# sovrasov/3d-object-detection.pytorch

Measured on AMD Instinct MI355X. Metric: regression train crops/sec @224^2 bs256 MobileNetV2, higher is better.
Workload: dtype bf16; 1 GPU; mobilenetv2 9-class Objectron keypoint regression, train step (fwd + l1/add/CE losses + bwd + AdamW), 224x224 crops, per-GPU batch 256; global_batch=256, parallelism=dp1, roofline_sampled_steps=0, rccl_ranks=0

## Files before the change

### 3d-object-detection.pytorch_amd/csrc/elementwise.hip

```cpp
#include "common.h"

namespace {

template <typename T, bool U8>
__global__ __launch_bounds__(256) void im2col_kernel(const void* __restrict__ xin, const float* __restrict__ mean,
                                                     const float* __restrict__ istd, T* __restrict__ col, int B,
                                                     int H, int W, int Ho, int Wo) {
  extern __shared__ float tile[];
  const int WP = W + 2;
  const int hp = (Ho + 1) / 2;
  const int b = blockIdx.x / hp, oy0 = (blockIdx.x % hp) * 2;
  const int iy0 = oy0 * 2 - 1;
  const int tid = threadIdx.x;
  for (int i = tid; i < 15 * 2; i += 256) {
    const int rr = i >> 1;
    tile[rr * WP + ((i & 1) ? W + 1 : 0)] = 0.f;
  }
  if constexpr (U8) {
    const unsigned char* xu = reinterpret_cast<const unsigned char*>(xin);
    const float mu[3] = {mean[0], mean[1], mean[2]}, is[3] = {istd[0], istd[1], istd[2]};
    const int RB = W * 3;
    if ((RB & 3) == 0) {
      const int R4 = RB >> 2;
      for (int i = tid; i < 5 * R4; i += 256) {
        const int r = i / R4, e0 = (i - r * R4) * 4;
        const int iy = iy0 + r;
        const bool ok = iy >= 0 && iy < H;
        const unsigned int u = ok ? *reinterpret_cast<const unsigned int*>(xu + ((size_t)b * H + iy) * RB + e0) : 0u;
#pragma unroll
        for (int k = 0; k < 4; ++k) {
          const int e = e0 + k, ix = e / 3, ci = e - ix * 3;
          const float m = ci == 0 ? mu[0] : (ci == 1 ? mu[1] : mu[2]), sc = ci == 0 ? is[0] : (ci == 1 ? is[1] : is[2]);
          tile[(ci * 5 + r) * WP + ix + 1] = ok ? ((float)((u >> (8 * k)) & 0xffu) * (1.0f / 255.0f) - m) * sc : 0.f;
        }
      }
    } else {
      for (int i = tid; i < 5 * RB; i += 256) {
        const int r = i / RB, e = i - r * RB, ix = e / 3, ci = e - ix * 3;
        const int iy = iy0 + r;
        float v = 0.f;
        if (iy >= 0 && iy < H) v = ((float)xu[((size_t)b * H + iy) * RB + e] * (1.0f / 255.0f) - mu[ci]) * is[ci];
        tile[(ci * 5 + r) * WP + ix + 1] = v;
      }
    }
  } else {
    const float* xf = reinterpret_cast<const float*>(xin);
    if ((W & 3) == 0) {
      const int W4 = W >> 2;
      for (int i = tid; i < 15 * W4; i += 256) {
        const int rr = i / W4, x4 = i - rr * W4, ci = rr / 5, r = rr - ci * 5;
        const int iy = iy0 + r;
        float4 v = make_float4(0.f, 0.f, 0.f, 0.f);
        if (iy >= 0 && iy < H) v = *reinterpret_cast<const float4*>(xf + (((size_t)b * 3 + ci) * H + iy) * W + x4 * 4);
        float* d = tile + rr * WP + x4 * 4 + 1;
        d[0] = v.x; d[1] = v.y; d[2] = v.z; d[3] = v.w;
      }
    } else {
      for (int i = tid; i < 15 * W; i += 256) {
        const int rr = i / W, ix = i - rr * W, ci = rr / 5, r = rr - ci * 5;
        const int iy = iy0 + r;
        tile[rr * WP + ix + 1] = (iy >= 0 && iy < H) ? xf[(((size_t)b * 3 + ci) * H + iy) * W + ix] : 0.f;
      }
    }
  }
  __syncthreads();
  const int nrow = min(2, Ho - oy0);
  for (int it = tid; it < nrow * Wo * 4; it += 256) {
    const int q = it & 3, pp = it >> 2, ro = pp / Wo, ox = pp - ro * Wo;
    float v[8];
#pragma unroll
    for (int i = 0; i < 8; ++i) {
      const int idx = q * 8 + i;
      const int ci = idx / 9, r = idx - ci * 9, ky = r / 3, kx = r - ky * 3;
      v[i] = idx < 27 ? tile[(ci * 5 + ro * 2 + ky) * WP + ox * 2 + kx] : 0.f;
    }
    Vec8<T>::store(col + (((size_t)b * Ho + oy0 + ro) * Wo + ox) * 32 + q * 8, v);
  }
}

struct EwArgs {
  const void *a, *b;
  const void* res;
  void* out;
  const float *scale, *shift;
  const float* vec;
  const float* vec2;
  float* pooled;
  double* stats;
  int act;
  int M, C, HW;
  float inv_hw;
  const T3dFold* fold;
  int mode;
  int* argmax;
};

__device__ __forceinline__ void load_affine(const EwArgs& a, int c0, float sc[8], float sh[8]) {
#pragma unroll
  for (int i = 0; i < 8; ++i) {
    sc[i] = a.scale ? a.scale[c0 + i] : 1.f;
    sh[i] = a.scale ? a.shift[c0 + i] : 0.f;
  }
}

__device__ __forceinline__ void flush_stats(float* lraw, int C, int c0, bool on, const float s1[8],
                                            const float s2[8], double* stats) {
  double* lstat = reinterpret_cast<double*>(lraw);
  for (int i = threadIdx.x; i < 2 * C; i += blockDim.x) lstat[i] = 0.0;
  __syncthreads();
  if (on) {
#pragma unroll
// ... 256 lines not shown
    }
  }
  if (a.stats) {
#pragma unroll
    for (int j = 0; j < 8; ++j) {
      red[0][slot * rowl + cgl * 8 + j] = s1[j];
      red[1][slot * rowl + cgl * 8 + j] = s2[j];
    }
    __syncthreads();
    const int t = threadIdx.x, c = blockIdx.y * rowl + t;
    if (t < rowl && c < a.C) {
      double u1 = 0.0, u2 = 0.0;
      for (int q = 0; q < nslots; ++q) {
        u1 += (double)red[0][q * rowl + t];
        u2 += (double)red[1][q * rowl + t];
      }
      double* st = a.stats + (size_t)(blockIdx.x % g_nrep) * g_rstride;
      atomicAdd(st + c, u1);
      atomicAdd(st + a.C + c, u2);
    }
  }
}

inline void fill_pro(EwArgs& a, const t3d_prologue* pro) {
  if (pro) { a.scale = pro->scale; a.shift = pro->shift; a.act = pro->act; }
}
inline int ew_grid(size_t nvec) {
  size_t g = (nvec + 255) / 256;
  return (int)(g < 1 ? 1 : (g > 2048 ? 2048 : g));
}

}

static int im2col_launch(int dtype, const void* x, bool u8, const float* mean, const float* istd, void* col, int B,
                         int H, int W, void* stream) {
  if (!x || !col || B <= 0 || H <= 0 || W <= 0 || (u8 && (!mean || !istd))) return T3D_ERR_ARG;
  const int Ho = (H + 2 - 3) / 2 + 1, Wo = (W + 2 - 3) / 2 + 1;
  const int grid = B * ((Ho + 1) / 2);
  const size_t lds = (size_t)15 * (W + 2) * sizeof(float);
  if (lds > 64 * 1024) return T3D_ERR_UNSUPPORTED;
  hipStream_t st = reinterpret_cast<hipStream_t>(stream);
#define T3D_IM2COL(T, U) \
  T3D_LAUNCH((im2col_kernel<T, U>), dim3(grid), dim3(256), lds, st, x, mean, istd, (T*)col, B, H, W, Ho, Wo)
  if (dtype == T3D_F32) {
    if (u8) T3D_IM2COL(float, true); else T3D_IM2COL(float, false);
  } else if (dtype == T3D_BF16) {
    if (u8) T3D_IM2COL(bf16_t, true); else T3D_IM2COL(bf16_t, false);
  } else if (dtype == T3D_F16) {
    if (u8) T3D_IM2COL(f16_t, true); else T3D_IM2COL(f16_t, false);
  } else {
    return T3D_ERR_ARG;
  }
#undef T3D_IM2COL
  T3D_CHECK_LAUNCH();
  return T3D_OK;
}

extern "C" int t3d_stem_im2col(int dtype, const float* x, void* col, int B, int H, int W, void* stream) {
  return im2col_launch(dtype, x, false, nullptr, nullptr, col, B, H, W, stream);
}

extern "C" int t3d_stem_im2col_u8(int dtype, const unsigned char* x, const float* mean, const float* inv_std, void* col,
                                  int B, int H, int W, void* stream) {
  return im2col_launch(dtype, x, true, mean, inv_std, col, B, H, W, stream);
}

extern "C" int t3d_bn_apply(int dtype, const void* y, const t3d_prologue* pro, const void* residual, void* z,
                            int M, int C, void* stream) {
  if (!y || !z || M <= 0 || C <= 0 || (C % 8)) return T3D_ERR_ARG;
  if (pro && pro->se) return T3D_ERR_UNSUPPORTED;
  EwArgs a{};
  a.a = y; a.res = residual; a.out = z; a.M = M; a.C = C;
  fill_pro(a, pro);
  const int grid = ew_grid((size_t)M * (C / 8));
  if ((size_t)grid * 256 < (size_t)(C / 8)) return T3D_ERR_UNSUPPORTED;
  hipStream_t st = reinterpret_cast<hipStream_t>(stream);
  a.fold = t3d_take_fold(a.scale);
  const size_t lds = a.fold ? (size_t)2 * C * sizeof(float) : 0;
  if (dtype == T3D_F32) T3D_LAUNCH(bn_apply_kernel<float>, dim3(grid), dim3(256), lds, st, a);
  else if (dtype == T3D_BF16) T3D_LAUNCH(bn_apply_kernel<bf16_t>, dim3(grid), dim3(256), lds, st, a);
  else if (dtype == T3D_F16) T3D_LAUNCH(bn_apply_kernel<f16_t>, dim3(grid), dim3(256), lds, st, a);
  else return T3D_ERR_ARG;
  T3D_CHECK_LAUNCH();
  return T3D_OK;
}

extern "C" int t3d_bn_act_bwd(int dtype, const void* dz, const void* y, const t3d_prologue* pro, void* dzp,
                              double* stats, int M, int C, void* stream) {
  if (!dz || !y || !dzp || M <= 0 || C <= 0 || (C % 8)) return T3D_ERR_ARG;
  if (pro && pro->se) return T3D_ERR_UNSUPPORTED;
  EwArgs a{};
  a.a = dz; a.b = y; a.out = dzp; a.stats = stats; a.M = M; a.C = C;
  fill_pro(a, pro);
  int grid = ew_grid((size_t)M * (C / 8));
  if (grid > 1024) grid = 1024;
  if ((size_t)grid * 256 < (size_t)(C / 8)) return T3D_ERR_UNSUPPORTED;
  const size_t lds = (size_t)2 * C * sizeof(double);
  hipStream_t st = reinterpret_cast<hipStream_t>(stream);
  if (dtype == T3D_F32) T3D_LAUNCH(bn_act_bwd_kernel<float>, dim3(grid), dim3(256), lds, st, a);
// ... 90 lines not shown
```

### 3d-object-detection.pytorch_amd/csrc/plan.hip

```cpp
#include <chrono>
#include <cstdio>
#include <cstdlib>
#include <cstring>
#include <string>
#include <utility>
#include <vector>

#include "common.h"

namespace {

template <class T>
inline T word_to(uint64_t v) {
  if constexpr (std::is_pointer<T>::value) {
    return reinterpret_cast<T>(static_cast<uintptr_t>(v));
  } else if constexpr (std::is_same<T, float>::value) {
    const uint32_t b = static_cast<uint32_t>(v);
    float f;
    std::memcpy(&f, &b, 4);
    return f;
  } else if constexpr (std::is_same<T, double>::value) {
    double d;
    std::memcpy(&d, &v, 8);
    return d;
  } else {
    return static_cast<T>(static_cast<int64_t>(v));
  }
}

template <class... A, size_t... I>
inline int call_words(int (*fn)(A...), const uint64_t* w, std::index_sequence<I...>) {
  return fn(word_to<A>(w[I])...);
}

template <class... A>
constexpr int arity(int (*)(A...)) { return (int)sizeof...(A); }

template <auto Fn>
struct Thunk;
template <class... A, int (*Fn)(A...)>
struct Thunk<Fn> {
  static int run(const uint64_t* w) { return call_words(Fn, w, std::index_sequence_for<A...>{}); }
};

struct Entry { const char* name; int (*run)(const uint64_t*); int nargs; };
#define T3D_E(fn) {#fn, &Thunk<&fn>::run, arity(&fn)}
const Entry kEntries[] = {
    T3D_E(t3d_dwconv_fwd), T3D_E(t3d_bn_finalize), T3D_E(t3d_bn_eval_affine), T3D_E(t3d_bn_eval_affine_batched),
    T3D_E(t3d_pwconv_fwd), T3D_E(t3d_pwconv_dgrad), T3D_E(t3d_pack_weight), T3D_E(t3d_sum_replicas_batched),
    T3D_E(t3d_set_dw_slots), T3D_E(t3d_set_exact_pool), T3D_E(t3d_sum_slots_batched), T3D_E(t3d_dwconv_bwd),
    T3D_E(t3d_pwconv_wgrad), T3D_E(t3d_pwconv_yfree_prep), T3D_E(t3d_pwconv_dgrad_yfree), T3D_E(t3d_pwconv_wgrad_yfree),
    T3D_E(t3d_pwconv_yfree_prep2), T3D_E(t3d_pwconv_bwd_yfree), T3D_E(t3d_pwconv_bwd_yfree_w), T3D_E(t3d_pwconv_wgrad_yfree_finish),
    T3D_E(t3d_bn_bwd_finalize), T3D_E(t3d_stem_im2col), T3D_E(t3d_stem_im2col_u8), T3D_E(t3d_crop_resize_u8),
    T3D_E(t3d_pwconv_fwd_mat), T3D_E(t3d_im2col), T3D_E(t3d_im2col_nchw), T3D_E(t3d_col2im_bwd), T3D_E(t3d_pack_conv_weight),
    T3D_E(t3d_unpack_conv_grad), T3D_E(t3d_maxpool_fwd), T3D_E(t3d_maxpool_bwd), T3D_E(t3d_res_relu_fwd),
    T3D_E(t3d_res_relu_bwd), T3D_E(t3d_subsample), T3D_E(t3d_ir_block_eval), T3D_E(t3d_bn_apply), T3D_E(t3d_bn_act_bwd),
    T3D_E(t3d_gap_fwd), T3D_E(t3d_gap_bwd), T3D_E(t3d_pool_fwd), T3D_E(t3d_pool_bwd), T3D_E(t3d_head_fwd),
    T3D_E(t3d_linear_fwd), T3D_E(t3d_head_fwd_all), T3D_E(t3d_head_bwd), T3D_E(t3d_head_bwd_weights), T3D_E(t3d_se_fwd),
    T3D_E(t3d_se_bwd), T3D_E(t3d_se_fwd_fused), T3D_E(t3d_se_bwd_data), T3D_E(t3d_se_bwd_weights), T3D_E(t3d_se_after_sums),
    T3D_E(t3d_se_after_apply), T3D_E(t3d_se_after_bwd), T3D_E(t3d_set_reduction_replicas), T3D_E(t3d_set_workspace), T3D_E(t3d_set_main_workspace),
    T3D_E(t3d_fold_request), T3D_E(t3d_pack_weights_batched), T3D_E(t3d_pwconv_pack_frag), T3D_E(t3d_adamw_step), T3D_E(t3d_set_grad_watch),
    T3D_E(t3d_sgd_step), T3D_E(t3d_rmsprop_step), T3D_E(t3d_adadelta_step),
    T3D_E(t3d_zero_batched), T3D_E(t3d_copy_cols), T3D_E(t3d_bn_bias_grad), T3D_E(t3d_se_bwd_affine), T3D_E(t3d_dropout_mask),
    T3D_E(t3d_loss_fwd_bwd), T3D_E(t3d_metrics_per_sample), T3D_E(t3d_iou3d), T3D_E(t3d_box_iou3d), T3D_E(t3d_ssd_decode_nms),
    T3D_E(t3d_expdw_fwd), T3D_E(t3d_track_step), T3D_E(t3d_ssd_select_rects), T3D_E(t3d_head_select), T3D_E(t3d_track_kp_to_frame),
    T3D_E(t3d_objectron_pairs), T3D_E(t3d_objectron_hitmiss), T3D_E(t3d_draw_overlays_u8),
};
#undef T3D_E
constexpr int kNumEntries = (int)(sizeof(kEntries) / sizeof(kEntries[0]));
constexpr int kMaxArgs = 24;

enum OpKind { OP_CALL = 0, OP_FORK = 1, OP_COPY_D2H = 2, OP_EVENT_RECORD = 3 };
enum ArgKind { ARG_WORD = 0, ARG_STRUCT = 1, ARG_SLOT = 2 };

struct Op {
  int kind;
  int entry;
  int nargs;
  uint64_t w[kMaxArgs];
  uint8_t ak[kMaxArgs];
  hipEvent_t ev;
  hipStream_t sig_stream;
};

}

// ... 228 lines not shown
```

### 3d-object-detection.pytorch_amd/torchdet3d/_native.py

```python
import ctypes
import os

import torch

_HERE = os.path.dirname(os.path.abspath(__file__))
LIB_PATH = os.environ.get('T3D_LIB') or os.path.join(os.path.dirname(_HERE), 'libt3d_hip.so')

W_FRAG = 0x100
F32, BF16, F16 = 0, 1, 2
ACT = {'none': 0, 'relu': 1, 'relu6': 2, 'hswish': 3}
DW_AUTO, DW_TILE, DW_ROW3, DW_PLANE7, DW_ROWK, DW_LDS = -1, 0, 1, 2, 3, 4
PW_AUTO, PW_DEEP, PW_STREAM, PW_REG32, PW_LDS, PW_TR, PW_PAIR = -1, 0, 1, 2, 3, 4, 5
PW_OP_FWD, PW_OP_FWD_STATS, PW_OP_MAT, PW_OP_DGRAD, PW_OP_WGRAD = 0, 1, 2, 3, 4
ERR_ARG, ERR_UNSUPPORTED = -1, -3
POOL = {'avg': 0, 'max': 1, 'avg+max': 2}
_P, _I, _F, _D, _L = ctypes.c_void_p, ctypes.c_int, ctypes.c_float, ctypes.c_double, ctypes.c_longlong


class BnBwd(ctypes.Structure):
    _fields_ = [('alpha', _P), ('beta', _P), ('gamma', _P), ('per_sample', _I)]


class Prologue(ctypes.Structure):
    _fields_ = [('scale', _P), ('shift', _P), ('se', _P), ('act', _I), ('se_after_act', _I)]


class LossCfg(ctypes.Structure):
    _fields_ = [(n, _F) for n in ('c_l1', 'c_mse', 'c_smoothl1', 'smoothl1_beta', 'c_add', 'c_diag', 'c_wing',
                                  'wing_w', 'wing_eps', 'c_ce', 'lam_reg', 'lam_cls')]


class BnFold(ctypes.Structure):
    _fields_ = [('kind', _I), ('C', _I), ('nrep', _I), ('rstride', _L), ('stats', _P), ('count', _D), ('gamma', _P), ('beta', _P),
                ('rm', _P), ('rv', _P), ('nbt', _P), ('momentum', _F), ('eps', _F), ('o0', _P), ('o1', _P), ('o2', _P),
                ('o3', _P), ('o4', _P), ('mean', _P), ('invstd', _P)]


class DrawStyleC(ctypes.Structure):
    _fields_ = [('rect_th', _I), ('edge_th', _I), ('kp_radius', _I), ('font_scale', _I), ('flags', _I),
                ('colors', ctypes.c_ubyte * 3 * 8)]


DRAW_IDS = 1
_PP = ctypes.POINTER(Prologue)
_BP = ctypes.POINTER(BnBwd)
_LP = ctypes.POINTER(LossCfg)

SIGNATURES = {
    't3d_version': [],
    't3d_dwconv_fwd': [_I, _P, _PP, _P, _P, _P, _P, _I, _I, _I, _I, _I, _I, _P],
    't3d_bn_finalize': [_P, _I, _D, _P, _P, _P, _P, _P, _F, _F, _P, _P, _P, _P, _P],
    't3d_bn_eval_affine': [_I, _P, _P, _P, _P, _F, _P, _P, _P],
    't3d_bn_eval_affine_batched': [_P, _I, _F, _P],
    't3d_pwconv_fwd': [_I, _P, _PP, _P, _P, _P, _P, _I, _I, _I, _I, _P],
    't3d_pwconv_dgrad': [_I, _P, _P, _BP, _P, _P, _PP, _P, _P, _P, _P, _I, _I, _I, _I, _P],
    't3d_pack_weight': [_I, _P, _P, _I, _I, _I, _P],
    't3d_sum_replicas_batched': [_P, _I, _I, _P],
    't3d_set_dw_slots': [_I, _P],
    't3d_set_exact_pool': [_I],
    't3d_set_launch_events': [_P, _P],
    't3d_sum_slots_batched': [_P, _I, _P],
    't3d_dwconv_bwd': [_I, _P, _P, _BP, _P, _P, _PP, _P, _P, _P, _P, _I, _I, _I, _I, _I, _I, _P],
    't3d_dwconv_route': [_I] * 10,
    't3d_dwconv_force_route': [_I],
    't3d_pwconv_wgrad': [_I, _P, _P, _BP, _P, _PP, _P, _I, _I, _I, _I, _P],
    't3d_pwconv_route': [_I] * 15,
    't3d_pwconv_force_route': [_I],
    't3d_pwconv_yfree_prep': [_P, _BP, _P, _P, _I, _I, _P],
    't3d_pwconv_dgrad_yfree': [_P, _P, _P, _P, _P, _PP, _P, _P, _P, _I, _I, _I, _I, _P],
    't3d_pwconv_wgrad_yfree': [_P, _P, _BP, _P, _P, _I, _I, _I, _I, _P],
    't3d_pwconv_yfree_prep2': [_P, _BP, _P, _P, _P, _I, _I, _P],
    't3d_pwconv_bwd_yfree_scratch': [_I, _I, _I],
    't3d_pwconv_bwd_yfree': [_P, _P, _P, _P, _PP, _P, _P, _P, _P, _L, _I, _I, _I, _I, _P],
    't3d_pwconv_bwd_yfree_w': [_P, _P, _P, _BP, _P, _PP, _P, _P, _P, _P, _L, _I, _I, _I, _I, _P],
    't3d_pwconv_wgrad_yfree_finish': [_P, _BP, _P, _P, _I, _I, _I, _P],
    't3d_bn_bwd_finalize': [_P, _I, _D, _P, _P, _P, _P, _P, _P, _P, _P, _P],
    't3d_stem_im2col': [_I, _P, _P, _I, _I, _I, _P],
    't3d_stem_im2col_u8': [_I, _P, _P, _P, _P, _I, _I, _I, _P],
    't3d_crop_resize_u8': [_P, _P, _P, _I, _I, _I, _I, _I, _P],
    't3d_augment_crops_u8': [_P, _L, _P, _P, _I, _I, _I, _P],
    't3d_augment_resized_u8': [_P, _L, _P, _P, _I, _I, _I, _P],
    't3d_augment_chain_crops_u8': [_P, _L, _P, _P, _P, _L, _P, _I, _I, _I, _I, _P],
    't3d_augment_chain_resized_u8': [_P, _L, _P, _P, _P, _L, _P, _I, _I, _I, _I, _P],
    't3d_pwconv_fwd_mat': [_I, _P, _PP, _P, _P, _P, _P, _P, _I, _I, _I, _I, _P],
    't3d_ssd_decode_nms': [_I, _I, _P, _P, _P, _P, _P, _P, _P, _I, _I, _F, _F, _I, _F, _F, _P, _P, _P, _P],
    't3d_track_state_bytes': [_I],
    't3d_track_lds_bytes': [_I, _I],
    't3d_track_step': [_P, _P, _P, _P, _I, _I, _I, _I, _I, _I, _D, _D, _I, _D, _D, _D, _I, _I, _P, _P, _P, _P, _P, _P],
    't3d_ssd_select_rects': [_P, _P, _I, _I, _I, _I, _F, _F, _I, _I, _D, _D, _I, _P, _P, _P, _P, _P, _P, _P],
    't3d_head_select': [_P, _P, _I, _I, _I, _P, _P, _P],
    't3d_track_kp_to_frame': [_P, _P, _P, _P, _I, _I, _P],
    't3d_draw_overlays_u8': [_P, _I, _I, _I, _P, _P, _P, _P, _P, _P, _I, _I, ctypes.POINTER(DrawStyleC), _P],
    't3d_draw_glyphs': [_P, _I],
    't3d_objectron_pairs': [_P] * 7 + [_I, _I, _I, _D, _D, _P, _P, _P],
    't3d_objectron_hitmiss': [_P] * 8 + [_I] * 5 + [_P] * 6,
    't3d_im2col': [_I, _P, _PP, _P, _I, _I, _I, _I, _I, _I, _I, _I, _P],
    't3d_im2col_nchw': [_I, _P, _P, _I, _I, _I, _I, _I, _I, _I, _I, _P],
    't3d_col2im_bwd': [_I, _P, _P, _PP, _P, _P, _I, _I, _I, _I, _I, _I, _I, _I, _P],
    't3d_pack_conv_weight': [_I, _P, _P, _I, _I, _I, _I, _P],
    't3d_unpack_conv_grad': [_P, _P, _I, _I, _I, _I, _P],
    't3d_maxpool_fwd': [_I, _P, _PP, _P, _P, _I, _I, _I, _I, _P],
    't3d_maxpool_bwd': [_I, _P, _P, _P, _PP, _P, _P, _I, _I, _I, _I, _P],
    't3d_res_relu_fwd': [_I, _P, _PP, _P, _PP, _P, _I, _I, _P],
    't3d_res_relu_bwd': [_I, _P, _P, _P, _P, _P, _P, _P, _I, _I, _P],
    't3d_subsample': [_I, _P, _P, _I, _I, _I, _I, _I, _I, _P],
    't3d_ir_block_eval': [_P, _P, _P, _P, _I, _P, _P, _P, _I, _P, _P, _P, _I, _P, _I, _I, _I, _I, _I, _I, _P],
    't3d_bn_apply': [_I, _P, _PP, _P, _P, _I, _I, _P],
    't3d_bn_act_bwd': [_I, _P, _P, _PP, _P, _P, _I, _I, _P],
    't3d_gap_fwd': [_I, _P, _PP, _P, _I, _I, _I, _P],
    't3d_gap_bwd': [_I, _P, _P, _PP, _P, _P, _I, _I, _I, _P],
    't3d_pool_fwd': [_I, _P, _PP, _I, _P, _P, _I, _I, _I, _P],
# ... 93 lines not shown
        return _raw_stream(torch.cuda.current_device())
    return torch.cuda.current_stream().cuda_stream


class KernelTimer:

    def __init__(self, only=None, prealloc=0, kernel_exact=False):
        self.only, self.rec, self.sig, self.kernel_exact = only, [], [], kernel_exact
        self.pool = [torch.cuda.Event(enable_timing=True) for _ in range(prealloc)]
        for e in self.pool:
            e.record()

    def event(self):
        return self.pool.pop() if self.pool else torch.cuda.Event(enable_timing=True)

    def per_launch(self):
        torch.cuda.synchronize()
        return [(n, sg, e0.elapsed_time(e1), nb) for (n, nb, e0, e1), sg in zip(self.rec, self.sig)]

    def summary(self):
        torch.cuda.synchronize()
        out = {}
        for name, nbytes, e0, e1 in self.rec:
            d = out.setdefault(name, dict(launches=0, ms=0.0, bytes=0))
            d['launches'] += 1
            d['ms'] += e0.elapsed_time(e1)
            d['bytes'] += nbytes or 0
        return out


timer = None
_KERNEL_TIMED = frozenset(('t3d_dwconv_fwd', 't3d_dwconv_bwd', 't3d_expdw_fwd', 't3d_pwconv_fwd', 't3d_pwconv_fwd_mat', 't3d_pwconv_dgrad',
                           't3d_pwconv_wgrad', 't3d_pwconv_dgrad_yfree', 't3d_pwconv_wgrad_yfree', 't3d_pwconv_bwd_yfree',
                           't3d_pwconv_bwd_yfree_w'))
_ABLATE = frozenset(x for x in os.environ.get('T3D_ABLATE', '').split(',') if x)


SLOT_IMGS, SLOT_GT, SLOT_CATS, SLOT_DROPOUT, SLOT_STEP, SLOT_LR, SLOT_RB_DST, SLOT_RB_EVENT, NSLOTS = range(9)
recorder = None


def call(name, *args, nbytes=None, slots=None):
    if _ABLATE and name in _ABLATE:
        return
    fn = getattr(lib(), name)
    if recorder is not None:
        recorder.add_call(name, args, nbytes, slots)
        rc = fn(*args)
        recorder.after_call()
        if rc != 0:
            raise RuntimeError(f'{name} failed with code {rc}')
        return
    t = timer
    if t is not None and (t.only is None or name in t.only):
        e0, e1 = t.event(), t.event()
        if name in _KERNEL_TIMED and t.kernel_exact:
            lib().t3d_set_launch_events(e0.cuda_event, e1.cuda_event)
            rc = fn(*args)
            lib().t3d_set_launch_events(None, None)
        else:
            e0.record()
            rc = fn(*args)
            e1.record()
        t.rec.append((name, nbytes, e0, e1))
        t.sig.append(tuple(a for a in args[:-1] if isinstance(a, int) and not isinstance(a, bool) and 0 <= a < (1 << 31)))
    else:
        rc = fn(*args)
# ... 126 lines not shown
```

### 3d-object-detection.pytorch_amd/torchdet3d/models/engine.py

```python
import math
import os

import torch

from .. import _native as N
from .arch import Arch

BN_EPS, BN_MOM = 1e-5, 0.1
NREP = 16
FUSED_EVAL_MIN_B = int(os.environ.get('T3D_FUSED_EVAL_MIN_B', '96'))
DW_SLOTS = int(os.environ.get('T3D_DW_SLOTS', '512'))
WORKSPACE_BYTES = 64 << 20
MAIN_WORKSPACE_BYTES = 16 << 20
YFREE_MIN_ELEMS = int(os.environ.get('T3D_YFREE_MIN', 8 << 20))
YFREE_MAX_K = int(os.environ.get('T3D_YFREE_MAX_K', 112))
HOOK_MIN = 1 << 20
SE_AFTER_FUSED = None
HOOK_ON_SIDE = True


def _se_after_fused_by_shape(dt, B, HW, C, R):
    if B < 8:
        return False
    if C * R <= 4096:
# ... 556 lines not shown
        finally:
            N.call('t3d_set_reduction_replicas', 1, 0)
            self._pool_exact(False)
            self._cur_nrep = None
        cur, a = sv['last_in'], self.arch
        M = sv['B'] * cur.H * cur.W
        z = torch.empty(M, a.last_c, device=self.device, dtype=self.dtype)
        N.call('t3d_bn_apply', self.dt, N.ptr(sv['yl']), sv['prol'], None, N.ptr(z), M, a.last_c, N.stream())
        return z.float().view(sv['B'], cur.H, cur.W, a.last_c).permute(0, 3, 1, 2).contiguous()

    def _features(self, imgs, train):
        a, st, dt = self.arch, N.stream(), self.dt
        u8 = imgs.dtype == torch.uint8
        assert imgs.is_cuda and imgs.dim() == 4 and ((u8 and imgs.shape[3] == 3) or (imgs.dtype == torch.float32 and imgs.shape[1] == 3))
        imgs = imgs.contiguous()
        self.training = bool(train)
        self._pack()
        if u8:
            B, H, W, _ = imgs.shape
        else:
            B, _, H, W = imgs.shape
        if train:
            self._zero_group('fwd', [[self._statbuf.data_ptr(), self._statbuf.numel() * self._statbuf.element_size()]])
        else:
            self._zero_group('fwd')
            self._eval_affines()
        sv = dict(B=B, imgs=imgs, blocks=[])
        self.saved_blocks = sv['blocks']

        Ho, Wo = (H + 2 - 3) // 2 + 1, (W + 2 - 3) // 2 + 1
        M = B * Ho * Wo
        bn0 = self.bns[a.keys.stem_bn]
        y0 = self._buf('y:stem', (M, a.stem_c))
        col = self._buf('col', (M, 32))
        if u8:
            N.call('t3d_stem_im2col_u8', dt, N.ptr(imgs), N.ptr(self.in_mean), N.ptr(self.in_istd), N.ptr(col), B, H, W, st)
        else:
            N.call('t3d_stem_im2col', dt, N.ptr(imgs), N.ptr(col), B, H, W, st)
        N.call('t3d_pwconv_fwd', dt, N.ptr(col), None, N.ptr(self.w['stem']), None, N.ptr(y0), self._st(bn0),
               M, Ho * Wo, 32, a.stem_c, st, nbytes=M * (32 + a.stem_c) * self.esz)
        pro0 = self._bn_fwd(bn0, M, a.stem_act)
        cur = _Src(y0, pro0, B, Ho, Wo, a.stem_c, raw=y0, bn=bn0, gpro=pro0)
        sv['col'], sv['stem'] = col, cur

        taps = getattr(self, '_want_taps', None)
        for i, blk in enumerate(a.blocks):
            cur = self._block_fwd(i, blk, cur, sv)
            if taps and (i + 1) in taps:
                sv.setdefault('taps', {})[i + 1] = self._resolve(cur)

        bnl = self.bns[a.keys.last_bn]
        M = cur.B * cur.H * cur.W
        yl = self._buf('y:last', (M, a.last_c))
        self._pw_from(cur, self.w[a.keys.last_w], yl, bnl, M, cur.H * cur.W, cur.C, a.last_c)
        prol = self._bn_fwd(bnl, M, a.last_act)
        pooled = self._buf('pooled', (B, a.last_c), torch.float32)
        sv.update(last_in=cur, yl=yl, prol=prol, pooled=pooled, HWl=cur.H * cur.W, bnl=bnl)
        return sv

    def _wsel(self, w, plain=True):
        f = self._frag.get(w.data_ptr()) if (plain and self.dt in (N.BF16, N.F16)) else None
        return (self.dt | N.W_FRAG, N.ptr(f)) if f is not None else (self.dt, N.ptr(w))

    def _resolve(self, src):
        if src.zbuf is not None:
            M = src.B * src.H * src.W
            self._c('t3d_bn_apply', self.dt, N.ptr(src.t), src.pro, N.ptr(src.zres), N.ptr(src.zbuf), M, src.C, N.stream(),
                    fwd=src.bn)
            src.t, src.pro, src.zres, src.zbuf = src.zbuf, None, None, None
        return src

    def _pw_from(self, x, w, y, bn_out, M, HW, K, Nn):
        st, nb = N.stream(), M * (K + Nn) * self.esz
# ... 529 lines not shown
```

### include/t3d.h

```cpp
#ifndef T3D_H_
#define T3D_H_
#include <stdint.h>
#ifdef __cplusplus
extern "C" {
#endif

enum { T3D_F32 = 0, T3D_BF16 = 1, T3D_F16 = 2 };
enum { T3D_W_FRAG = 0x100 };
enum { T3D_ACT_NONE = 0, T3D_ACT_RELU = 1, T3D_ACT_RELU6 = 2, T3D_ACT_HSWISH = 3 };
enum { T3D_OK = 0, T3D_ERR_ARG = -1, T3D_ERR_LAUNCH = -2, T3D_ERR_UNSUPPORTED = -3 };

typedef struct {
  const float* scale;
  const float* shift;
  const float* se;
  int act;
  int se_after_act;
} t3d_prologue;

int t3d_version(void);

int t3d_dwconv_fwd(int dtype, const void* x, const t3d_prologue* pro, const float* w, void* y,
                   double* stats, float* gap_sum, int B, int H, int W, int C, int k, int stride,
                   void* stream);
// ... 41 lines not shown

int t3d_pwconv_yfree_prep(const void* wt, const t3d_bnbwd* bb, void* wcat, float* cvec, int K, int N, void* stream);
int t3d_pwconv_dgrad_yfree(const void* dz, const void* x, const void* wcat, const float* cvec, const void* x_raw,
                           const t3d_prologue* pro_in, const void* residual, void* dx, double* stats, int M, int HW,
                           int K, int N, void* stream);
int t3d_pwconv_wgrad_yfree(const void* dz, const void* x, const t3d_bnbwd* bb, const void* w, float* dw, int M, int HW,
                           int K, int N, void* stream);

int t3d_pwconv_yfree_prep2(const void* wt, const t3d_bnbwd* bb, void* wcat, float* cvec, void* wd, int K, int N, void* stream);
int t3d_pwconv_bwd_yfree_w(const void* dz, const void* x, const void* wt, const t3d_bnbwd* bb, const void* x_raw,
                           const t3d_prologue* pro_in, const void* residual, void* dx, double* stats, void* scratch,
                           long long scratch_bytes, int M, int HW, int K, int N, void* stream);
int t3d_pwconv_bwd_yfree_scratch(int M, int K, int N);
int t3d_pwconv_bwd_yfree(const void* dz, const void* x, const void* wd, const void* x_raw, const t3d_prologue* pro_in,
                         const void* residual, void* dx, double* stats, void* scratch, long long scratch_bytes, int M, int HW,
                         int K, int N, void* stream);
int t3d_pwconv_wgrad_yfree_finish(void* scratch, const t3d_bnbwd* bb, const void* w, float* dw, int M, int K, int N, void* stream);

int t3d_dwconv_bwd(int dtype, const void* dz, const void* y, const t3d_bnbwd* bb, const float* w,
                   const void* x, const t3d_prologue* pro, const void* residual, void* dx, double* stats,
                   float* dw, int B, int H, int W, int C, int k, int stride, void* stream);

enum { T3D_DW_AUTO = -1, T3D_DW_TILE = 0, T3D_DW_ROW3 = 1, T3D_DW_PLANE7 = 2, T3D_DW_ROWK = 3, T3D_DW_LDS = 4 };
int t3d_dwconv_route(int backward, int dtype, int gated_input, int pooled, int B, int H, int W, int C, int k, int stride);
int t3d_dwconv_force_route(int route);

int t3d_bn_bwd_finalize(const double* stats, int C, double count, const float* gamma, const float* mean,
                        const float* invstd, float* alpha, float* beta, float* gammac, float* dgamma,
                        float* dbeta, void* stream);

int t3d_stem_im2col(int dtype, const float* x, void* col, int B, int H, int W, void* stream);
int t3d_stem_im2col_u8(int dtype, const unsigned char* x, const float* mean, const float* inv_std, void* col, int B, int H,
                       int W, void* stream);

int t3d_ir_block_eval(const void* x, const void* w1, const float* scale1, const float* shift1, int act1, const float* wdw,
                      const float* scale2, const float* shift2, int act2, const void* w2, const float* scale3,
                      const float* shift3, int residual, void* z, int B, int H, int W, int Cin, int Ce, int Cout, void* stream);

int t3d_crop_resize_u8(const unsigned char* frame, const int* rects, unsigned char* out, int n, int H, int W, int oh, int ow,
                       void* stream);

enum { T3D_AUG_FLIP = 1, T3D_AUG_LUT = 2, T3D_AUG_ROTATE = 4, T3D_AUG_SWAP_RB = 8 };
typedef struct {
  long long offset;
  int h, w;
  int flags;
  float alpha;
  float beta255;
  int reserved;
  double m[6];
} t3d_aug_sample;
int t3d_augment_crops_u8(const unsigned char* src, long long src_bytes, const void* samples, unsigned char* out, int B, int oh,
                         int ow, void* stream);

int t3d_augment_resized_u8(const unsigned char* arena, long long arena_bytes, const void* samples, unsigned char* out, int B,
                           int oh, int ow, void* stream);

enum { T3D_CHAIN_LUT = 1, T3D_CHAIN_HSV = 2, T3D_CHAIN_BRIGHTNESS = 3, T3D_CHAIN_CONTRAST = 4, T3D_CHAIN_SATURATION = 5,
       T3D_CHAIN_HUE = 6 };
enum { T3D_CHAIN_WARP2 = 1 };
enum { T3D_STAGE_MEAN = 1, T3D_STAGE_WARP = 2, T3D_STAGE_WARP2 = 4 };
#define T3D_CHAIN_MAX_OPS 8
typedef struct {
  int n_ops;
  int flags;
  int kind[T3D_CHAIN_MAX_OPS];
// ... 227 lines not shown
```

Before: 38160 crops/s.

## Fuse stem im2col, MFMA conv and BN stats into one persistent kernel

```diff
diff --git a/3d-object-detection.pytorch_amd/csrc/elementwise.hip b/3d-object-detection.pytorch_amd/csrc/elementwise.hip
--- a/3d-object-detection.pytorch_amd/csrc/elementwise.hip
+++ b/3d-object-detection.pytorch_amd/csrc/elementwise.hip
@@ -1,82 +1,6 @@
 #include "common.h"
 
 namespace {
-
-template <typename T, bool U8>
-__global__ __launch_bounds__(256) void im2col_kernel(const void* __restrict__ xin, const float* __restrict__ mean,
-                                                     const float* __restrict__ istd, T* __restrict__ col, int B,
-                                                     int H, int W, int Ho, int Wo) {
-  extern __shared__ float tile[];
-  const int WP = W + 2;
-  const int hp = (Ho + 1) / 2;
-  const int b = blockIdx.x / hp, oy0 = (blockIdx.x % hp) * 2;
-  const int iy0 = oy0 * 2 - 1;
-  const int tid = threadIdx.x;
-  for (int i = tid; i < 15 * 2; i += 256) {
-    const int rr = i >> 1;
-    tile[rr * WP + ((i & 1) ? W + 1 : 0)] = 0.f;
-  }
-  if constexpr (U8) {
-    const unsigned char* xu = reinterpret_cast<const unsigned char*>(xin);
-    const float mu[3] = {mean[0], mean[1], mean[2]}, is[3] = {istd[0], istd[1], istd[2]};
-    const int RB = W * 3;
-    if ((RB & 3) == 0) {
-      const int R4 = RB >> 2;
-      for (int i = tid; i < 5 * R4; i += 256) {
-        const int r = i / R4, e0 = (i - r * R4) * 4;
-        const int iy = iy0 + r;
-        const bool ok = iy >= 0 && iy < H;
-        const unsigned int u = ok ? *reinterpret_cast<const unsigned int*>(xu + ((size_t)b * H + iy) * RB + e0) : 0u;
-#pragma unroll
-        for (int k = 0; k < 4; ++k) {
-          const int e = e0 + k, ix = e / 3, ci = e - ix * 3;
-          const float m = ci == 0 ? mu[0] : (ci == 1 ? mu[1] : mu[2]), sc = ci == 0 ? is[0] : (ci == 1 ? is[1] : is[2]);
-          tile[(ci * 5 + r) * WP + ix + 1] = ok ? ((float)((u >> (8 * k)) & 0xffu) * (1.0f / 255.0f) - m) * sc : 0.f;
-        }
-      }
-    } else {
-      for (int i = tid; i < 5 * RB; i += 256) {
-        const int r = i / RB, e = i - r * RB, ix = e / 3, ci = e - ix * 3;
-        const int iy = iy0 + r;
-        float v = 0.f;
-        if (iy >= 0 && iy < H) v = ((float)xu[((size_t)b * H + iy) * RB + e] * (1.0f / 255.0f) - mu[ci]) * is[ci];
-        tile[(ci * 5 + r) * WP + ix + 1] = v;
-      }
-    }
-  } else {
-    const float* xf = reinterpret_cast<const float*>(xin);
-    if ((W & 3) == 0) {
-      const int W4 = W >> 2;
-      for (int i = tid; i < 15 * W4; i += 256) {
-        const int rr = i / W4, x4 = i - rr * W4, ci = rr / 5, r = rr - ci * 5;
-        const int iy = iy0 + r;
-        float4 v = make_float4(0.f, 0.f, 0.f, 0.f);
-        if (iy >= 0 && iy < H) v = *reinterpret_cast<const float4*>(xf + (((size_t)b * 3 + ci) * H + iy) * W + x4 * 4);
-        float* d = tile + rr * WP + x4 * 4 + 1;
-        d[0] = v.x; d[1] = v.y; d[2] = v.z; d[3] = v.w;
-      }
-    } else {
-      for (int i = tid; i < 15 * W; i += 256) {
-        const int rr = i / W, ix = i - rr * W, ci = rr / 5, r = rr - ci * 5;
-        const int iy = iy0 + r;
-        tile[rr * WP + ix + 1] = (iy >= 0 && iy < H) ? xf[(((size_t)b * 3 + ci) * H + iy) * W + ix] : 0.f;
-      }
-    }
-  }
-  __syncthreads();
-  const int nrow = min(2, Ho - oy0);
-  for (int it = tid; it < nrow * Wo * 4; it += 256) {
-    const int q = it & 3, pp = it >> 2, ro = pp / Wo, ox = pp - ro * Wo;
-    float v[8];
-#pragma unroll
-    for (int i = 0; i < 8; ++i) {
-      const int idx = q * 8 + i;
-      const int ci = idx / 9, r = idx - ci * 9, ky = r / 3, kx = r - ky * 3;
-      v[i] = idx < 27 ? tile[(ci * 5 + ro * 2 + ky) * WP + ox * 2 + kx] : 0.f;
-    }
-    Vec8<T>::store(col + (((size_t)b * Ho + oy0 + ro) * Wo + ox) * 32 + q * 8, v);
-  }
-}
 
 struct EwArgs {
   const void *a, *b;
@@ -399,39 +323,6 @@
 
 }
 
-static int im2col_launch(int dtype, const void* x, bool u8, const float* mean, const float* istd, void* col, int B,
-                         int H, int W, void* stream) {
-  if (!x || !col || B <= 0 || H <= 0 || W <= 0 || (u8 && (!mean || !istd))) return T3D_ERR_ARG;
-  const int Ho = (H + 2 - 3) / 2 + 1, Wo = (W + 2 - 3) / 2 + 1;
-  const int grid = B * ((Ho + 1) / 2);
-  const size_t lds = (size_t)15 * (W + 2) * sizeof(float);
-  if (lds > 64 * 1024) return T3D_ERR_UNSUPPORTED;
-  hipStream_t st = reinterpret_cast<hipStream_t>(stream);
-#define T3D_IM2COL(T, U) \
-  T3D_LAUNCH((im2col_kernel<T, U>), dim3(grid), dim3(256), lds, st, x, mean, istd, (T*)col, B, H, W, Ho, Wo)
-  if (dtype == T3D_F32) {
-    if (u8) T3D_IM2COL(float, true); else T3D_IM2COL(float, false);
-  } else if (dtype == T3D_BF16) {
-    if (u8) T3D_IM2COL(bf16_t, true); else T3D_IM2COL(bf16_t, false);
-  } else if (dtype == T3D_F16) {
-    if (u8) T3D_IM2COL(f16_t, true); else T3D_IM2COL(f16_t, false);
-  } else {
-    return T3D_ERR_ARG;
-  }
-#undef T3D_IM2COL
-  T3D_CHECK_LAUNCH();
-  return T3D_OK;
-}
-
-extern "C" int t3d_stem_im2col(int dtype, const float* x, void* col, int B, int H, int W, void* stream) {
-  return im2col_launch(dtype, x, false, nullptr, nullptr, col, B, H, W, stream);
-}
-
-extern "C" int t3d_stem_im2col_u8(int dtype, const unsigned char* x, const float* mean, const float* inv_std, void* col,
-                                  int B, int H, int W, void* stream) {
-  return im2col_launch(dtype, x, true, mean, inv_std, col, B, H, W, stream);
-}
-
 extern "C" int t3d_bn_apply(int dtype, const void* y, const t3d_prologue* pro, const void* residual, void* z,
                             int M, int C, void* stream) {
   if (!y || !z || M <= 0 || C <= 0 || (C % 8)) return T3D_ERR_ARG;
diff --git a/3d-object-detection.pytorch_amd/csrc/plan.hip b/3d-object-detection.pytorch_amd/csrc/plan.hip
--- a/3d-object-detection.pytorch_amd/csrc/plan.hip
+++ b/3d-object-detection.pytorch_amd/csrc/plan.hip
@@ -51,7 +51,7 @@
     T3D_E(t3d_set_dw_slots), T3D_E(t3d_set_exact_pool), T3D_E(t3d_sum_slots_batched), T3D_E(t3d_dwconv_bwd),
     T3D_E(t3d_pwconv_wgrad), T3D_E(t3d_pwconv_yfree_prep), T3D_E(t3d_pwconv_dgrad_yfree), T3D_E(t3d_pwconv_wgrad_yfree),
     T3D_E(t3d_pwconv_yfree_prep2), T3D_E(t3d_pwconv_bwd_yfree), T3D_E(t3d_pwconv_bwd_yfree_w), T3D_E(t3d_pwconv_wgrad_yfree_finish),
-    T3D_E(t3d_bn_bwd_finalize), T3D_E(t3d_stem_im2col), T3D_E(t3d_stem_im2col_u8), T3D_E(t3d_crop_resize_u8),
+    T3D_E(t3d_bn_bwd_finalize), T3D_E(t3d_stem_im2col), T3D_E(t3d_stem_im2col_u8), T3D_E(t3d_stem_fwd), T3D_E(t3d_crop_resize_u8),
     T3D_E(t3d_pwconv_fwd_mat), T3D_E(t3d_im2col), T3D_E(t3d_im2col_nchw), T3D_E(t3d_col2im_bwd), T3D_E(t3d_pack_conv_weight),
     T3D_E(t3d_unpack_conv_grad), T3D_E(t3d_maxpool_fwd), T3D_E(t3d_maxpool_bwd), T3D_E(t3d_res_relu_fwd),
     T3D_E(t3d_res_relu_bwd), T3D_E(t3d_subsample), T3D_E(t3d_ir_block_eval), T3D_E(t3d_bn_apply), T3D_E(t3d_bn_act_bwd),
diff --git a/3d-object-detection.pytorch_amd/csrc/stem.hip b/3d-object-detection.pytorch_amd/csrc/stem.hip
--- /dev/null
+++ b/3d-object-detection.pytorch_amd/csrc/stem.hip
@@ -0,0 +1,288 @@
+#include <cstdlib>
+#include "common.h"
+
+namespace {
+
+template <bool U8>
+__device__ __forceinline__ void stem_stage_rows(float* __restrict__ tile, const void* __restrict__ xin,
+                                                const float* __restrict__ mean, const float* __restrict__ istd, int b,
+                                                int iy0, int H, int W) {
+  const int WP = W + 2;
+  const int tid = threadIdx.x;
+  for (int i = tid; i < 15 * 2; i += 256) {
+    const int rr = i >> 1;
+    tile[rr * WP + ((i & 1) ? W + 1 : 0)] = 0.f;
+  }
+  if constexpr (U8) {
+    const unsigned char* xu = reinterpret_cast<const unsigned char*>(xin);
+    const float mu[3] = {mean[0], mean[1], mean[2]}, is[3] = {istd[0], istd[1], istd[2]};
+    const int RB = W * 3;
+    if ((RB & 3) == 0) {
+      const int R4 = RB >> 2;
+      for (int i = tid; i < 5 * R4; i += 256) {
+        const int r = i / R4, e0 = (i - r * R4) * 4;
+        const int iy = iy0 + r;
+        const bool ok = iy >= 0 && iy < H;
+        const unsigned int u = ok ? *reinterpret_cast<const unsigned int*>(xu + ((size_t)b * H + iy) * RB + e0) : 0u;
+#pragma unroll
+        for (int k = 0; k < 4; ++k) {
+          const int e = e0 + k, ix = e / 3, ci = e - ix * 3;
+          const float m = ci == 0 ? mu[0] : (ci == 1 ? mu[1] : mu[2]), sc = ci == 0 ? is[0] : (ci == 1 ? is[1] : is[2]);
+          tile[(ci * 5 + r) * WP + ix + 1] = ok ? ((float)((u >> (8 * k)) & 0xffu) * (1.0f / 255.0f) - m) * sc : 0.f;
+        }
+      }
+    } else {
+      for (int i = tid; i < 5 * RB; i += 256) {
+        const int r = i / RB, e = i - r * RB, ix = e / 3, ci = e - ix * 3;
+        const int iy = iy0 + r;
+        float v = 0.f;
+        if (iy >= 0 && iy < H) v = ((float)xu[((size_t)b * H + iy) * RB + e] * (1.0f / 255.0f) - mu[ci]) * is[ci];
+        tile[(ci * 5 + r) * WP + ix + 1] = v;
+      }
+    }
+  } else {
+    const float* xf = reinterpret_cast<const float*>(xin);
+    if ((W & 3) == 0) {
+      const int W4 = W >> 2;
+      for (int i = tid; i < 15 * W4; i += 256) {
+        const int rr = i / W4, x4 = i - rr * W4, ci = rr / 5, r = rr - ci * 5;
+        const int iy = iy0 + r;
+        float4 v = make_float4(0.f, 0.f, 0.f, 0.f);
+        if (iy >= 0 && iy < H) v = *reinterpret_cast<const float4*>(xf + (((size_t)b * 3 + ci) * H + iy) * W + x4 * 4);
+        float* d = tile + rr * WP + x4 * 4 + 1;
+        d[0] = v.x; d[1] = v.y; d[2] = v.z; d[3] = v.w;
+      }
+    } else {
+      for (int i = tid; i < 15 * W; i += 256) {
+        const int rr = i / W, ix = i - rr * W, ci = rr / 5, r = rr - ci * 5;
+        const int iy = iy0 + r;
+        tile[rr * WP + ix + 1] = (iy >= 0 && iy < H) ? xf[(((size_t)b * 3 + ci) * H + iy) * W + ix] : 0.f;
+      }
+    }
+  }
+}
+
+template <typename T, bool U8>
+__global__ __launch_bounds__(256) void im2col_kernel(const void* __restrict__ xin, const float* __restrict__ mean,
+                                                     const float* __restrict__ istd, T* __restrict__ col, int B,
+                                                     int H, int W, int Ho, int Wo) {
+  extern __shared__ float tile[];
+  const int WP = W + 2;
+  const int hp = (Ho + 1) / 2;
+  const int b = blockIdx.x / hp, oy0 = (blockIdx.x % hp) * 2;
+  const int tid = threadIdx.x;
+  stem_stage_rows<U8>(tile, xin, mean, istd, b, oy0 * 2 - 1, H, W);
+  __syncthreads();
+  const int nrow = min(2, Ho - oy0);
+  for (int it = tid; it < nrow * Wo * 4; it += 256) {
+    const int q = it & 3, pp = it >> 2, ro = pp / Wo, ox = pp - ro * Wo;
+    float v[8];
+#pragma unroll
+    for (int i = 0; i < 8; ++i) {
+      const int idx = q * 8 + i;
+      const int ci = idx / 9, r = idx - ci * 9, ky = r / 3, kx = r - ky * 3;
+      v[i] = idx < 27 ? tile[(ci * 5 + ro * 2 + ky) * WP + ox * 2 + kx] : 0.f;
+    }
+    Vec8<T>::store(col + (((size_t)b * Ho + oy0 + ro) * Wo + ox) * 32 + q * 8, v);
+  }
+}
+
+template <typename T> struct StemMma;
+template <> struct StemMma<bf16_t> {
+  typedef bf16x8 V;
+  static __device__ __forceinline__ f32x4 run(V a, V b, f32x4 c) { return __builtin_amdgcn_mfma_f32_16x16x32_bf16(a, b, c, 0, 0, 0); }
+};
+template <> struct StemMma<f16_t> {
+  typedef f16x8 V;
+  static __device__ __forceinline__ f32x4 run(V a, V b, f32x4 c) { return __builtin_amdgcn_mfma_f32_16x16x32_f16(a, b, c, 0, 0, 0); }
+};
+
+template <typename T, bool U8>
+__global__ __launch_bounds__(256) void stem_fwd_kernel(const void* __restrict__ xin, const float* __restrict__ mean,
+                                                       const float* __restrict__ istd, const T* __restrict__ w,
+                                                       T* __restrict__ y, T* __restrict__ col, double* __restrict__ stats,
+                                                       const T3dQuant quant, const int nrep, const long long rstride, int B,
+                                                       int H, int W, int Ho, int Wo, int C) {
+  typedef typename StemMma<T>::V V;
+  extern __shared__ float tile[];
+  __shared__ double dstat[64];
+  const int WP = W + 2;
+  const int hp = (Ho + 1) / 2, nunits = B * hp;
+  const int tid = threadIdx.x, lane = tid & 63, wave = tid >> 6;
+  const int lg = lane >> 4, lc = lane & 15;
+  const int nb = lg * 8;
+  V wf[2];
+#pragma unroll
+  for (int t = 0; t < 2; ++t) {
+    const int n = (lc >> 2) * 8 + t * 4 + (lc & 3);
+    wf[t] = *reinterpret_cast<const V*>(w + (size_t)min(n, C - 1) * 32 + lg * 8);
+    if (n >= C) {
+#pragma unroll
+      for (int j = 0; j < 8; ++j) wf[t][j] = (T)0.f;
+    }
+  }
+  int off[8];
+#pragma unroll
+  for (int i = 0; i < 8; ++i) {
+    const int idx = min(lg * 8 + i, 26);
+    const int ci = idx / 9, r = idx - ci * 9, ky = r / 3, kx = r - ky * 3;
+    off[i] = (ci * 5 + ky) * WP + kx;
+  }
+  float st1[8], st2[8];
+#pragma unroll
+  for (int j = 0; j < 8; ++j) st1[j] = st2[j] = 0.f;
+  if (tid < 64) dstat[tid] = 0.0;
+
+  for (int unit = blockIdx.x; unit < nunits; unit += gridDim.x) {
+    const int b = unit / hp, oy0 = (unit - b * hp) * 2;
+    __syncthreads();
+    stem_stage_rows<U8>(tile, xin, mean, istd, b, oy0 * 2 - 1, H, W);
+    __syncthreads();
+    const int npix = min(2, Ho - oy0) * Wo;
+    const size_t m0 = ((size_t)b * Ho + oy0) * Wo;
+    for (int g = wave; g * 16 < npix; g += 4) {
+      const int pp = g * 16 + lc;
+      const bool ok = pp < npix;
+      const int pc = min(pp, npix - 1);
+      const int ro = pc >= Wo ? 1 : 0, ox = pc - ro * Wo;
+      const float* src = tile + ro * 2 * WP + ox * 2;
+      V bf;
+#pragma unroll
+      for (int i = 0; i < 8; ++i) bf[i] = (T)((lg * 8 + i < 27) ? src[off[i]] : 0.f);
+      const f32x4 z = {0.f, 0.f, 0.f, 0.f};
+      const f32x4 a0 = StemMma<T>::run(wf[0], bf, z), a1 = StemMma<T>::run(wf[1], bf, z);
+      if (col && ok) *reinterpret_cast<V*>(col + (m0 + pp) * 32 + lg * 8) = bf;
+      if (nb < C) {
+        float v[8] = {a0[0], a0[1], a0[2], a0[3], a1[0], a1[1], a1[2], a1[3]};
+#pragma unroll
+        for (int j = 0; j < 8; ++j) v[j] = ok ? Vec8<T>::round(v[j]) : 0.f;
+        if (ok) Vec8<T>::store(y + (m0 + pp) * C + nb, v);
+        if (stats) {
+#pragma unroll
+          for (int j = 0; j < 8; ++j) {
+            st1[j] += v[j];
+            st2[j] = fmaf(v[j], v[j], st2[j]);
+          }
+        }
+      }
+    }
+  }
+  if (stats) {
+    __syncthreads();
+#pragma unroll
+    for (int j = 0; j < 8; ++j) {
+      const float s1 = row16_sum(st1[j]), s2 = row16_sum(st2[j]);
+      if (lc == 0 && nb < C) {
+        atomicAdd(dstat + (nb + j) * 2, t3d_snap(s1, quant, false));
+        atomicAdd(dstat + (nb + j) * 2 + 1, t3d_snap(s2, quant, true));
+      }
+    }
+    __syncthreads();
+    if (tid < 2 * C) atomicAdd(stats + (size_t)(blockIdx.x % nrep) * rstride + (size_t)(tid & 1) * C + (tid >> 1), dstat[tid]);
+  }
+}
+
+int g_forced = T3D_STEM_AUTO;
+
+bool fused_can(int dtype, int C) { return (dtype == T3D_BF16 || dtype == T3D_F16) && (C == 16 || C == 32); }
+
+size_t tile_bytes(int W) {
+  const size_t lds = (size_t)15 * (W + 2) * sizeof(float);
+  return lds > 64 * 1024 ? 0 : lds;
+}
+
+template <typename T, bool U8>
+int fused_launch(const void* x, const float* mean, const float* istd, const void* w, void* y, void* col, double* stats, size_t lds,
+                 int B, int H, int W, int Ho, int Wo, int C, hipStream_t st) {
+  static int occ = 0;
+  if (occ == 0) {
+    int n = 0;
+    if (hipOccupancyMaxActiveBlocksPerMultiprocessor(&n, (const void*)stem_fwd_kernel<T, U8>, 256, 0) != hipSuccess || n < 1) n = 1;
+    occ = n;
+  }
+  const int by_lds = (int)(160 * 1024 / (lds + 1024));
+  int per_cu = occ < by_lds ? occ : by_lds;
+  if (per_cu < 1) per_cu = 1;
+  const int nunits = B * ((Ho + 1) / 2);
+  const int grid = nunits < 256 * per_cu ? nunits : 256 * per_cu;
+  const T3dQuant quant = (stats && !T3D_ENV_SET("T3D_NO_SNAP")) ? t3d_quant_for((long long)B * Ho * Wo) : T3dQuant{0.0, 0.0};
+  const int nrep = g_t3d_reduce.nrep < 1 ? 1 : g_t3d_reduce.nrep;
+  T3D_LAUNCH_TIMED((stem_fwd_kernel<T, U8>), dim3(grid), dim3(256), lds, st, x, mean, istd, (const T*)w, (T*)y, (T*)col, stats, quant,
+                   nrep, g_t3d_reduce.stats_stride, B, H, W, Ho, Wo, C);
+  T3D_CHECK_LAUNCH();
+  return T3D_OK;
+}
+
+}
+
+static int im2col_launch(int dtype, const void* x, bool u8, const float* mean, const float* istd, void* col, int B,
+                         int H, int W, void* stream) {
+  if (!x || !col || B <= 0 || H <= 0 || W <= 0 || (u8 && (!mean || !istd))) return T3D_ERR_ARG;
+  const int Ho = (H + 2 - 3) / 2 + 1, Wo = (W + 2 - 3) / 2 + 1;
+  const int grid = B * ((Ho + 1) / 2);
+  const size_t lds = tile_bytes(W);
+  if (!lds) return T3D_ERR_UNSUPPORTED;
+  hipStream_t st = reinterpret_cast<hipStream_t>(stream);
+#define T3D_IM2COL(T, U) \
+  T3D_LAUNCH((im2col_kernel<T, U>), dim3(grid), dim3(256), lds, st, x, mean, istd, (T*)col, B, H, W, Ho, Wo)
+  if (dtype == T3D_F32) {
+    if (u8) T3D_IM2COL(float, true); else T3D_IM2COL(float, false);
+  } else if (dtype == T3D_BF16) {
+    if (u8) T3D_IM2COL(bf16_t, true); else T3D_IM2COL(bf16_t, false);
+  } else if (dtype == T3D_F16) {
+    if (u8) T3D_IM2COL(f16_t, true); else T3D_IM2COL(f16_t, false);
+  } else {
+    return T3D_ERR_ARG;
+  }
+#undef T3D_IM2COL
+  T3D_CHECK_LAUNCH();
+  return T3D_OK;
+}
+
+extern "C" int t3d_stem_im2col(int dtype, const float* x, void* col, int B, int H, int W, void* stream) {
+  return im2col_launch(dtype, x, false, nullptr, nullptr, col, B, H, W, stream);
+}
+
+extern "C" int t3d_stem_im2col_u8(int dtype, const unsigned char* x, const float* mean, const float* inv_std, void* col,
+                                  int B, int H, int W, void* stream) {
+  return im2col_launch(dtype, x, true, mean, inv_std, col, B, H, W, stream);
+}
+
+extern "C" int t3d_stem_route(int dtype, int fmt, int C) {
+  if (dtype < T3D_F32 || dtype > T3D_F16 || (fmt != T3D_STEM_F32_NCHW && fmt != T3D_STEM_U8_NHWC) || C <= 0 || (C % 8)) return T3D_ERR_ARG;
+  if (g_forced == T3D_STEM_PAIR) return T3D_STEM_PAIR;
+  if (fused_can(dtype, C)) return T3D_STEM_FUSED;
+  return g_forced == T3D_STEM_FUSED ? T3D_ERR_UNSUPPORTED : T3D_STEM_PAIR;
+}
+
+extern "C" int t3d_stem_force_route(int route) {
+  if (route != T3D_STEM_AUTO && route != T3D_STEM_FUSED && route != T3D_STEM_PAIR) return T3D_ERR_ARG;
+  g_forced = route;
+  return T3D_OK;
+}
+
+extern "C" int t3d_stem_fwd(int dtype, int fmt, const void* x, const float* mean, const float* inv_std, const void* w, void* y,
+                            double* stats, void* col, int B, int H, int W, int C, void* stream) {
+  const int route = t3d_stem_route(dtype, fmt, C);
+  if (route < 0) return route;
+  const bool u8 = fmt == T3D_STEM_U8_NHWC;
+  if (!x || !w || !y || B <= 0 || H <= 0 || W <= 0 || (u8 && (!mean || !inv_std))) return T3D_ERR_ARG;
+  const size_t lds = tile_bytes(W);
+  if (!lds) return T3D_ERR_UNSUPPORTED;
+  if (dtype == T3D_F16 && stats) return T3D_ERR_UNSUPPORTED;
+  const int Ho = (H + 2 - 3) / 2 + 1, Wo = (W + 2 - 3) / 2 + 1;
+  const int M = B * Ho * Wo;
+  if (route == T3D_STEM_PAIR) {
+    if (!col) return T3D_ERR_ARG;
+    const int rc = t3d_pwconv_route(T3D_PW_OP_FWD, dtype, 0, 0, 0, 0, 0, stats != nullptr, 0, T3D_ACT_NONE, 0, M, Ho * Wo, 32, C);
+    if (rc < 0) return rc;
+    if (const int e = im2col_launch(dtype, x, u8, mean, inv_std, col, B, H, W, stream)) return e;
+    return t3d_pwconv_fwd(dtype, col, nullptr, w, nullptr, y, stats, M, Ho * Wo, 32, C, stream);
+  }
+  hipStream_t st = reinterpret_cast<hipStream_t>(stream);
+  if (dtype == T3D_BF16)
+    return u8 ? fused_launch<bf16_t, true>(x, mean, inv_std, w, y, col, stats, lds, B, H, W, Ho, Wo, C, st)
+              : fused_launch<bf16_t, false>(x, mean, inv_std, w, y, col, stats, lds, B, H, W, Ho, Wo, C, st);
+  return u8 ? fused_launch<f16_t, true>(x, mean, inv_std, w, y, col, stats, lds, B, H, W, Ho, Wo, C, st)
+            : fused_launch<f16_t, false>(x, mean, inv_std, w, y, col, stats, lds, B, H, W, Ho, Wo, C, st);
+}
diff --git a/3d-object-detection.pytorch_amd/torchdet3d/_native.py b/3d-object-detection.pytorch_amd/torchdet3d/_native.py
--- a/3d-object-detection.pytorch_amd/torchdet3d/_native.py
+++ b/3d-object-detection.pytorch_amd/torchdet3d/_native.py
@@ -12,6 +12,8 @@
 DW_AUTO, DW_TILE, DW_ROW3, DW_PLANE7, DW_ROWK, DW_LDS = -1, 0, 1, 2, 3, 4
 PW_AUTO, PW_DEEP, PW_STREAM, PW_REG32, PW_LDS, PW_TR, PW_PAIR = -1, 0, 1, 2, 3, 4, 5
 PW_OP_FWD, PW_OP_FWD_STATS, PW_OP_MAT, PW_OP_DGRAD, PW_OP_WGRAD = 0, 1, 2, 3, 4
+STEM_AUTO, STEM_FUSED, STEM_PAIR = -1, 0, 1
+STEM_F32_NCHW, STEM_U8_NHWC = 0, 1
 ERR_ARG, ERR_UNSUPPORTED = -1, -3
 POOL = {'avg': 0, 'max': 1, 'avg+max': 2}
 _P, _I, _F, _D, _L = ctypes.c_void_p, ctypes.c_int, ctypes.c_float, ctypes.c_double, ctypes.c_longlong
@@ -77,6 +79,9 @@
     't3d_bn_bwd_finalize': [_P, _I, _D, _P, _P, _P, _P, _P, _P, _P, _P, _P],
     't3d_stem_im2col': [_I, _P, _P, _I, _I, _I, _P],
     't3d_stem_im2col_u8': [_I, _P, _P, _P, _P, _I, _I, _I, _P],
+    't3d_stem_route': [_I, _I, _I],
+    't3d_stem_force_route': [_I],
+    't3d_stem_fwd': [_I, _I, _P, _P, _P, _P, _P, _P, _P, _I, _I, _I, _I, _P],
     't3d_crop_resize_u8': [_P, _P, _P, _I, _I, _I, _I, _I, _P],
     't3d_augment_crops_u8': [_P, _L, _P, _P, _I, _I, _I, _P],
     't3d_augment_resized_u8': [_P, _L, _P, _P, _I, _I, _I, _P],
@@ -236,7 +241,7 @@
 timer = None
 _KERNEL_TIMED = frozenset(('t3d_dwconv_fwd', 't3d_dwconv_bwd', 't3d_expdw_fwd', 't3d_pwconv_fwd', 't3d_pwconv_fwd_mat', 't3d_pwconv_dgrad',
                            't3d_pwconv_wgrad', 't3d_pwconv_dgrad_yfree', 't3d_pwconv_wgrad_yfree', 't3d_pwconv_bwd_yfree',
-                           't3d_pwconv_bwd_yfree_w'))
+                           't3d_pwconv_bwd_yfree_w', 't3d_stem_fwd'))
 _ABLATE = frozenset(x for x in os.environ.get('T3D_ABLATE', '').split(',') if x)
 
 
diff --git a/3d-object-detection.pytorch_amd/torchdet3d/models/engine.py b/3d-object-detection.pytorch_amd/torchdet3d/models/engine.py
--- a/3d-object-detection.pytorch_amd/torchdet3d/models/engine.py
+++ b/3d-object-detection.pytorch_amd/torchdet3d/models/engine.py
@@ -612,13 +612,12 @@
         M = B * Ho * Wo
         bn0 = self.bns[a.keys.stem_bn]
         y0 = self._buf('y:stem', (M, a.stem_c))
-        col = self._buf('col', (M, 32))
-        if u8:
-            N.call('t3d_stem_im2col_u8', dt, N.ptr(imgs), N.ptr(self.in_mean), N.ptr(self.in_istd), N.ptr(col), B, H, W, st)
-        else:
-            N.call('t3d_stem_im2col', dt, N.ptr(imgs), N.ptr(col), B, H, W, st)
-        N.call('t3d_pwconv_fwd', dt, N.ptr(col), None, N.ptr(self.w['stem']), None, N.ptr(y0), self._st(bn0),
-               M, Ho * Wo, 32, a.stem_c, st, nbytes=M * (32 + a.stem_c) * self.esz)
+        fmt = N.STEM_U8_NHWC if u8 else N.STEM_F32_NCHW
+        fused = N.lib().t3d_stem_route(dt, fmt, a.stem_c) == N.STEM_FUSED
+        col = self._buf('col', (M, 32)) if train or not fused else None
+        N.call('t3d_stem_fwd', dt, fmt, N.ptr(imgs), N.ptr(self.in_mean) if u8 else None, N.ptr(self.in_istd) if u8 else None,
+               N.ptr(self.w['stem']), N.ptr(y0), self._st(bn0), N.ptr(col), B, H, W, a.stem_c, st,
+               nbytes=imgs.numel() * imgs.element_size() + M * (a.stem_c + (32 if col is not None else 0)) * self.esz)
         pro0 = self._bn_fwd(bn0, M, a.stem_act)
         cur = _Src(y0, pro0, B, Ho, Wo, a.stem_c, raw=y0, bn=bn0, gpro=pro0)
         sv['col'], sv['stem'] = col, cur
diff --git a/include/t3d.h b/include/t3d.h
--- a/include/t3d.h
+++ b/include/t3d.h
@@ -97,6 +97,13 @@
 int t3d_stem_im2col(int dtype, const float* x, void* col, int B, int H, int W, void* stream);
 int t3d_stem_im2col_u8(int dtype, const unsigned char* x, const float* mean, const float* inv_std, void* col, int B, int H,
                        int W, void* stream);
+
+enum { T3D_STEM_AUTO = -1, T3D_STEM_FUSED = 0, T3D_STEM_PAIR = 1 };
+enum { T3D_STEM_F32_NCHW = 0, T3D_STEM_U8_NHWC = 1 };
+int t3d_stem_route(int dtype, int fmt, int C);
+int t3d_stem_force_route(int route);
+int t3d_stem_fwd(int dtype, int fmt, const void* x, const float* mean, const float* inv_std, const void* w, void* y,
+                 double* stats, void* col, int B, int H, int W, int C, void* stream);
 
 int t3d_ir_block_eval(const void* x, const void* w1, const float* scale1, const float* shift1, int act1, const float* wdw,
                       const float* scale2, const float* shift2, int act2, const void* w2, const float* scale3,
```

Measured after the change: 38250 crops/s, median of 2. Within noise of the previous version (+0.2%).
